# yardenas/ethz-safe-learning

Hardware: AMD Instinct MI355X
Metric: planning steps/sec (CEM-MPC, N=2000 K=5 H=30) (higher is better)
Workload: dtype f32

## Files before the change

### ethz_safe_learning_amd/_capi.py

```python
from __future__ import annotations

import ctypes as C
import os

CEM_ABI_VERSION = 4
CEM_MAX_ACT = 32
CEM_MAX_COST_KINDS = 4
CEM_COMM_ID_BYTES = 128
CEM_MAX_BATCH = 256
CEM_TRAIN_MAX_BATCH = 4096
CEM_INIT_COLD, CEM_INIT_EXPLICIT, CEM_INIT_SHIFT = 0, 1, 2
CEM_VARIANT_CEM, CEM_VARIANT_SAFE, CEM_VARIANT_COST = 0, 1, 2
CEM_PARTICLES_MEAN, CEM_PARTICLES_LOWER_TAIL = 0, 1
CEM_CONSTRAINT_BETA, CEM_CONSTRAINT_BUDGET = 0, 1
CEM_REFIT_UNIFORM, CEM_REFIT_SOFTMAX = 0, 1
CEM_NOISE_WHITE, CEM_NOISE_MIXED = 0, 1
CEM_FORWARD_SPLIT, CEM_FORWARD_ALL = 0, 1
CEM_TASK_SAFETY_GYM, CEM_TASK_QUADRATIC = 0, 1

_HERE = os.path.dirname(os.path.abspath(__file__))
LIB_PATH = os.environ.get('CEM_MPC_LIB') or os.path.join(_HERE, 'lib', 'libcem_mpc_gfx950.so')

EXPORTED_SYMBOLS = [
    'cem_abi_version', 'cem_status_string', 'cem_last_hip_error', 'cem_weight_blob_floats',
    'cem_packed_weight_floats', 'cem_workspace_bytes', 'cem_pack_weights_host', 'cem_plan_tiles_host', 'cem_plan_segments_host', 'cem_rollout_residency',
    'cem_planner_create', 'cem_planner_destroy', 'cem_planner_layout', 'cem_planner_set_weights', 'cem_planner_set_weights_dev',
    'cem_planner_set_normaliser', 'cem_planner_plan', 'cem_plan_begin', 'cem_plan_rollout', 'cem_plan_select',
    'cem_plan_end', 'cem_comm_unique_id', 'cem_planner_comm_init', 'cem_planner_comm_destroy', 'cem_planner_comm_ranks', 'cem_plan_exchange', 'cem_planner_graph_status', 'cem_planner_graph_nodes', 'cem_planner_launches_per_iteration', 'cem_planner_rollout_path', 'cem_planner_rollout_form', 'cem_unfold_sequences', 'cem_compute_objective', 'cem_scorer_reward', 'cem_scorer_cost', 'cem_fill_noise', 'cem_philox_words', 'cem_planner_set_timing', 'cem_planner_last_timing', 'cem_planner_last_timing_detail', 'cem_planner_select_mode', 'cem_planner_inject_fault',
    'cem_batch_workspace_bytes', 'cem_batch_planner_create', 'cem_planner_plan_batch', 'cem_planner_batch_capacity',
    'cem_planner_set_warm_start', 'cem_planner_set_initial_distribution', 'cem_planner_set_init_mode', 'cem_planner_reset_carry',
    'cem_planner_get_carry', 'cem_planner_set_carry_slots', 'cem_planner_set_particle_objective', 'cem_planner_get_particle_objective',
    'cem_planner_set_constraint', 'cem_planner_get_constraint', 'cem_planner_set_cost_budget', 'cem_planner_constraint_costs',
    'cem_planner_set_refit', 'cem_planner_get_refit', 'cem_planner_refit_stats',
    'cem_planner_set_action_noise', 'cem_planner_get_action_noise', 'cem_planner_action_noise_dev',
    'cem_planner_set_elite_carry', 'cem_planner_get_elite_carry', 'cem_planner_elite_store',
    'cem_planner_set_population_schedule', 'cem_planner_get_population_schedule', 'cem_planner_iteration_plan',
    'cem_planner_set_mean_candidate', 'cem_planner_get_mean_candidate',
    'cem_planner_set_plan_readout', 'cem_planner_get_plan_readout', 'cem_planner_plan_readout',
    'cem_planner_set_task', 'cem_planner_task_trajectories', 'cem_task_score',
    'cem_trainer_workspace_bytes', 'cem_trainer_blob_floats', 'cem_trainer_create', 'cem_trainer_destroy', 'cem_trainer_set_state',
    'cem_trainer_get_state', 'cem_trainer_weights_dev', 'cem_trainer_step', 'cem_trainer_steps', 'cem_trainer_eval', 'cem_trainer_forward',
]

# ... 109 lines not shown
    lib.cem_planner_comm_init.argtypes = [vp, vp, C.c_int32, C.c_int32]
    lib.cem_planner_comm_destroy.argtypes = [vp]
    lib.cem_plan_exchange.argtypes = [vp]
    lib.cem_planner_graph_status.argtypes = [vp, i32p]
    lib.cem_planner_graph_nodes.argtypes = [vp, i32p]
    lib.cem_planner_comm_ranks.argtypes = [vp, i32p]
    lib.cem_planner_launches_per_iteration.argtypes = [vp, i32p]
    lib.cem_planner_rollout_path.argtypes = [vp, i32p]
    lib.cem_planner_rollout_form.argtypes = [vp, C.c_int32, i32p]
    lib.cem_compute_objective.argtypes = [vp, vp, C.c_int32, C.c_int32, vp]
    lib.cem_scorer_reward.argtypes = [vp, vp, vp, C.c_int32, vp, vp]
    lib.cem_scorer_cost.argtypes = [vp, vp, C.c_int32, vp]
    lib.cem_fill_noise.argtypes = [vp, C.c_uint64, C.c_uint64, vp, vp, vp]
    lib.cem_philox_words.argtypes = [vp, C.c_uint64, C.c_uint64] + [C.c_uint32] * 6 + [vp]
    lib.cem_planner_select_mode.argtypes = [vp, i32p]
    lib.cem_planner_inject_fault.argtypes = [vp, C.c_int32]
    lib.cem_planner_set_timing.argtypes = [vp, C.c_int32]
    lib.cem_planner_last_timing.argtypes = [vp, fp, i32p, fp]
    lib.cem_planner_last_timing_detail.argtypes = [vp, fp, fp]
    lib.cem_batch_workspace_bytes.restype = C.c_size_t
    lib.cem_batch_workspace_bytes.argtypes = [cfgp, C.c_int32]
    lib.cem_batch_planner_create.argtypes = [cfgp, C.c_int32, vp, C.c_size_t, vp, C.POINTER(vp)]
    lib.cem_planner_plan_batch.argtypes = [vp, C.c_int32, vp, C.c_uint64, vp, vp, vp, vp, vp, vp, vp]
    lib.cem_planner_batch_capacity.argtypes = [vp, i32p]
    lib.cem_planner_set_warm_start.argtypes = [vp, C.POINTER(CemWarmStart)]
    lib.cem_planner_set_initial_distribution.argtypes = [vp, C.c_int32, vp, vp]
    lib.cem_planner_set_init_mode.argtypes = [vp, C.c_int32, C.c_int32]
    lib.cem_planner_reset_carry.argtypes = [vp, C.c_int32]
    lib.cem_planner_get_carry.argtypes = [vp, C.c_int32, vp, vp, i32p]
    lib.cem_planner_set_carry_slots.argtypes = [vp, C.c_int32, vp]
# ... 54 lines not shown
```

### ethz_safe_learning_amd/csrc/cem_capi.hip

```cpp
#include "cem_device.h"
#include "cem_rollout_lean.h"
#include "cem_score.h"
#include "cem_refit_weighted.h"
#include "cem_noise_mix.h"
#include "cem_elite_carry.h"
#include "cem_plan_readout.h"
#include "cem_task_score.h"
#include "cem_population.h"
#include "cem_train.h"
#include "cem_train_tile.h"
#include "cem_forward.h"
#include "cem_rollout_split.h"
#include "cem_rollout_bf16.h"
#include "cem_rollout_wide.h"
#include "cem_pack.h"
#include "../../include/cem_mpc.h"
#include "cem_plan_options.h"

#include <dlfcn.h>
#include <link.h>

#include <algorithm>
#include <atomic>
#include <chrono>
// ... 602 lines not shown
struct cem_planner {
    cem_config_t cfg;
    Dims d;
    Layout lay;
    char *ws;
    hipStream_t stream;
    bool own_stream;
    int rc;
    int n_tiles;
    int n_seg, seg_len, n_pinned;
    bool have_weights;
    bool in_plan;
    bool sample_in_rollout;
    bool lean_rollout;
    bool lean_branchy;
    const float *eps_act, *eps_model;
    CtrlBlock *h_ctrl;
    float *h_result;
    WarmCtl *h_warm; const WarmCtl *d_h_warm;
    uint32_t plan_seq;
    const CtrlBlock *d_h_ctrl; float *d_h_result;
    bool timing; std::vector<hipEvent_t> ev; float roll_ms, sel_ms, red_ms, samp_ms; int roll_n;
    std::vector<std::pair<int, int>> ev_kind;
    hipGraph_t graph; hipGraphExec_t gexec; bool graph_ready;
    ScorerDev sc;
    ScorerDev sc_roll;
    float alpha, beta;
    void *comm;
    int plans_since_comm;
    bool graph_failed;
    size_t sel_dyn_limit;
    int fused_resident;
    bool sel_zeroed;
    bool fuse_banned;
    bool inject_capture_fail;
    uint32_t inject_next;
    char *scratch; size_t scratch_bytes;
    std::vector<float> h_etab;
    PackDesc *pack_desc; uint32_t n_pack_desc;
    int batch;
    int n_states;
    cem_warm_start_t warm;
    std::vector<int32_t> slot_mode;
    std::vector<uint8_t> carry_valid, have_expl;
    std::vector<int32_t> carry_at;
    std::vector<int32_t> slot_of;
// ... 51 lines not shown
    return straight ? 2 : 1;
}
size_t task_tab_floats() { return (size_t)CEM_TASK_TABLES * CEM_U; }
float *task_traj(const cem_planner *h) { return h->task_dev + task_tab_floats(); }
int32_t *elite_counts(const cem_planner *h) { return reinterpret_cast<int32_t *>(h->elite_dev); }
size_t elite_count_floats(const cem_planner *h) { return ((size_t)warm_slots(h) + 63) & ~(size_t)63; }
float *elite_store(const cem_planner *h) { return h->elite_dev + elite_count_floats(h); }

int select_mode_for(const cem_planner *h, int N, bool *cache = nullptr)
{
    const Dims &d = h->d;
    const bool can_fuse = (N + CEM_MS_KEYS - 1) / CEM_MS_KEYS <= h->fused_resident && !h->fuse_banned;
    return resolve_select_mode(h->cfg.select_mode, N, d.k, (long long)d.H * d.A, h->sel_dyn_limit, can_fuse, cache);
}
int select_mode_now(const cem_planner *h, bool *cache = nullptr) { return select_mode_for(h, h->d.N, cache); }

void drop_graph(cem_planner *h)
{
    if (h->gexec) { hipGraphExecDestroy(h->gexec); h->gexec = nullptr; }
    if (h->graph) { hipGraphDestroy(h->graph); h->graph = nullptr; }
    h->graph_ready = false;
}

struct LaunchRecipe {
    bool sampler_launch;
    bool inject_elites, inject_mean;
    int lean_form;
    bool fold_reduce;
    int select_mode; bool select_cache;
    bool one_workgroup_only;
    bool weighted, keep_elites, track;
    bool task;
};
LaunchRecipe recipe_of(const cem_planner *h, int it, bool own_noise)
{
    const IterView v = iter_view(h, it); const PlanOptions &o = h->opt;
    LaunchRecipe r{};
    r.inject_elites = o.elite.n_keep != 0;
    r.inject_mean = o.mean_cand && it == h->d.I - 1;
    r.task = o.task != 0;
    const bool rewritten = r.inject_elites || r.inject_mean || r.task;
    r.sampler_launch = !v.sample_in_rollout || rewritten;
    r.lean_form = v.lean_rollout && !rewritten && !own_noise && o.noise_kind != CEM_NOISE_MIXED ? lean_form(h, it) : 0;
    r.select_mode = select_mode_for(h, v.d->N, &r.select_cache);
    r.fold_reduce = h->d.W == 1 && !h->comm && h->cfg.variant == CEM_VARIANT_CEM && !o.tail_m && r.select_mode == 1 && r.select_cache;
    r.weighted = o.refit_kind == CEM_REFIT_SOFTMAX; r.keep_elites = o.elite.n_keep != 0; r.track = o.readout != 0;
    r.one_workgroup_only = r.weighted || r.keep_elites || r.track || !h->pop.empty();
    return r;
}

int launches_of(const cem_planner *h, int it)
{
    const LaunchRecipe r = recipe_of(h, it, false);
    return 1 + r.sampler_launch + r.inject_elites + r.inject_mean + !r.fold_reduce + (r.select_mode == 2 ? 8 : r.select_mode == 3 ? 2 : 1) +
           r.weighted + r.keep_elites + r.track + r.task;
}

PlanOptions options_of(const cem_planner *h) { PlanOptions o = h->opt; o.comm = h->comm != nullptr; return o; }

// ... 177 lines not shown
    cem_planner *h = new (std::nothrow) cem_planner();
    if (!h) return CEM_ERR_INVALID_ARG;
    h->cfg = *cfg; h->d = make_dims(cfg);
    h->batch = mb; h->n_states = warm_slots(h);
    const size_t nb = (size_t)warm_slots(h);
    h->lay = make_layout(cfg, h->d, max_tiles_of(h->d), mb);
    if (workspace_bytes < h->lay.total || ((uintptr_t)workspace & 255)) { delete h; return CEM_ERR_WORKSPACE; }
    h->ws = (char *)workspace; h->stream = (hipStream_t)hip_stream; h->own_stream = false;
    if (!h->stream) {
        if (hipStreamCreateWithFlags(&h->stream, hipStreamNonBlocking) != hipSuccess) { g_last_hip = (int)hipGetLastError(); delete h; return CEM_ERR_HIP; }
        h->own_stream = true;
    }
    { const Plan pl = make_plan(cfg, h->d, mb); h->rc = pl.rc; h->n_seg = pl.n_seg; h->seg_len = pl.seg_len; h->n_pinned = pl.n_pinned;
      place_sampler(h, h->d, pl, &h->sample_in_rollout, &h->lean_rollout); }
    { const char *e = std::getenv("CEM_FORCE_ROLLOUT"); h->lean_branchy = e && std::strcmp(e, "lean_branchy") == 0; }
    h->have_weights = false; h->in_plan = false; h->eps_act = h->eps_model = nullptr;
    h->timing = false; h->roll_ms = h->sel_ms = h->red_ms = h->samp_ms = 0.f; h->roll_n = 0;
    h->graph = nullptr; h->gexec = nullptr; h->graph_ready = false;
    h->budget_dev = nullptr; h->cstat_obj = nullptr; h->cstat_obj_n = 0; h->last_cstat = nullptr; h->last_cstat_n = h->last_cstat_problems = 0;
    h->refit_beta = 0.f; h->refit_dev = nullptr; h->refit_ran = false;
    h->noise_dev = nullptr; h->noise_eps = nullptr; h->noise_floats = 0;
    h->elite_dev = nullptr; h->elite_cap = 0; h->elite_clear = false;
    h->readout_dev = nullptr;
    h->task_dev = nullptr; h->task = TaskScoreParams{};
    h->pop_dev = nullptr; h->pop_seg_flags = nullptr; h->pop_seg_state = nullptr; h->pop_n_ready = 0;
    h->h_budget.assign(nb, std::numeric_limits<float>::infinity());
    h->comm = nullptr; h->plans_since_comm = 0; h->graph_failed = false;
    h->h_ctrl = nullptr; h->h_result = nullptr; h->h_warm = nullptr; h->d_h_warm = nullptr; h->pack_desc = nullptr; h->n_pack_desc = 0;
    h->warm = cem_warm_start_t{}; h->warm.shift = 1; h->warm_staged = 0; h->warm_save_skipped = false;
    h->slot_mode.assign(nb, CEM_INIT_COLD); h->carry_valid.assign(nb, 0); h->have_expl.assign(nb, 0); h->carry_at.assign(nb, -1);
// ... 71 lines not shown
        !upload(h->lay.tiles, tiles.data(), tiles.size() * sizeof(Tile6)) || !upload(h->lay.omask, om.data(), om.size() * 4) ||
        !upload(h->lay.kind_sel, ks.data(), ks.size() * 4) || !upload(h->lay.nmin, mn.data(), CEM_U * 4) ||
        !upload(h->lay.ndelta, dl.data(), CEM_U * 4) || !upload(h->lay.etab, h->h_etab.data(), h->h_etab.size() * 4) ||
        hipMemsetAsync(h->ws + h->lay.act_pad, 0, nb * d.N * d.H * d.act_nq * 16, h->stream) != hipSuccess ||
        hipStreamSynchronize(h->stream) != hipSuccess)
        return fail(CEM_ERR_HIP);

    h->sel_dyn_limit = 48 * 1024;
    if (hipFuncSetAttribute(reinterpret_cast<const void *>(&cem_select_kernel<true, false>), hipFuncAttributeMaxDynamicSharedMemorySize,
                            140 * 1024) == hipSuccess &&
        hipFuncSetAttribute(reinterpret_cast<const void *>(&cem_select_kernel<true, true>), hipFuncAttributeMaxDynamicSharedMemorySize,
                            140 * 1024) == hipSuccess &&
        hipFuncSetAttribute(reinterpret_cast<const void *>(&cem_select_kernel<false, false>), hipFuncAttributeMaxDynamicSharedMemorySize,
                            140 * 1024) == hipSuccess) h->sel_dyn_limit = 140 * 1024;
    else (void)hipGetLastError();
    {
        int per_cu = 0;
        if (hipOccupancyMaxActiveBlocksPerMultiprocessor(&per_cu, cem_msel_fused_kernel, 1024, 0) != hipSuccess || per_cu < 1) { (void)hipGetLastError(); per_cu = 0; }
        h->fused_resident = per_cu * real_cus();
    }
    if (mb && select_mode_now(h) != 1) { release_handle(h); return CEM_ERR_UNSUPPORTED; }
    *out = h;
    return CEM_OK;
}

extern "C" {

int cem_planner_create(const cem_config_t *cfg, void *workspace, size_t workspace_bytes, void *hip_stream, cem_planner_t **out)
{
    return planner_create(cfg, 0, workspace, workspace_bytes, hip_stream, out);
// ... 421 lines not shown
            hipLaunchKernelGGL(cem_msel_hist_kernel<2>, dim3(m.G), dim3(1024), 0, h->stream, m);
            hipLaunchKernelGGL(cem_msel_count_kernel, dim3(m.G), dim3(1024), 0, h->stream, m);
            hipLaunchKernelGGL(cem_msel_compact_kernel, dim3(m.G), dim3(1024), 0, h->stream, m);
            hipLaunchKernelGGL(cem_msel_moments_kernel<0>, dim3(m.G2), dim3(256), 0, h->stream, m);
            hipLaunchKernelGGL(cem_msel_moments_kernel<1>, dim3(m.G2), dim3(256), 0, h->stream, m);
            hipLaunchKernelGGL(cem_msel_final_kernel, dim3(1), dim3(256), 0, h->stream, m);
        }
    } else {
        if (fold_final && !h->batch && !weighted) {
            p.is_last = it == d.I - 1;
            p.result = h->d_h_result; p.result_dev = (uint32_t *)(ws + l.result); p.eps_out = have_eps_out ? (const float *)(ws + l.eps_out) : nullptr; p.noise_stddev = h->cfg.noise_stddev;
            if (folded) *folded = true;
        }
        if (cache) lds += (size_t)CEM_SEL_KWORDS(d.N) * 4;
        const dim3 grid(warm_slots(h));
        if (cache && h->cfg.variant != CEM_VARIANT_CEM) hipLaunchKernelGGL((cem_select_kernel<true, true>), grid, dim3(1024), lds, h->stream, p);
        else if (cache) hipLaunchKernelGGL((cem_select_kernel<true, false>), grid, dim3(1024), lds, h->stream, p);
        else hipLaunchKernelGGL((cem_select_kernel<false, false>), grid, dim3(1024), lds, h->stream, p);
        if (weighted) {
            HIPCHK(hipGetLastError());
            RefitWeightedParams rw{}; rw.scores = p.scores; rw.actions = p.actions; rw.musig = (float *)(ws + l.musig); rw.ctrl = p.ctrl; rw.elite_idx = p.elite_idx;
            rw.stat = h->refit_dev + (size_t)warm_slots(h) * 2 * p.HA;
            rw.N = d.N; rw.k = d.k; rw.HA = p.HA; rw.I = d.I; rw.beta = h->refit_beta;
            rw.smoothing = p.smoothing; rw.one_minus_smoothing = p.one_minus_smoothing; rw.threshold = h->cfg.stddev_threshold;
            HIPCHK(launch_refit_weighted(rw, warm_slots(h), h->stream));
            h->refit_ran = true;
        }
        if (rc.keep_elites) {
            HIPCHK(hipGetLastError());
            const EliteCarryParams ep = fill_elite(h, it);
            HIPCHK(launch_elite_keep(ep, warm_slots(h), h->stream));
// ... 1066 lines not shown
    WordsParams wp{}; wp.out = words_out_dev; wp.ctrl = (const CtrlBlock *)(h->ws + h->lay.ctrl);
    wp.stream = stream; wp.it = iteration; wp.t = t; wp.sub = sub; wp.idx0 = idx0; wp.n = n;
    hipLaunchKernelGGL(cem_philox_words_kernel, dim3((n + 255) / 256), dim3(256), 0, h->stream, wp);
    HIPCHK(hipGetLastError());
    HIPCHK(hipStreamSynchronize(h->stream));
    return CEM_OK;
}

int cem_planner_select_mode(const cem_planner_t *h, int32_t *mode_out)
{
    if (!h || !mode_out) return CEM_ERR_INVALID_ARG;
    *mode_out = select_mode_now(h);
    return CEM_OK;
}

int cem_planner_inject_fault(cem_planner_t *h, int32_t kind)
{
    if (!h || (kind != 1 && kind != 2)) return CEM_ERR_INVALID_ARG;
    if (h->in_plan) return CEM_ERR_STATE;
    if (kind == 2) { h->inject_capture_fail = true; return CEM_OK; }
    h->inject_next = 1u;
    return CEM_OK;
}

int cem_planner_set_timing(cem_planner_t *h, int32_t enable)
{
    if (!h) return CEM_ERR_INVALID_ARG;
    h->timing = enable != 0;
    return CEM_OK;
}
// ... 308 lines not shown
```

### ethz_safe_learning_amd/csrc/cem_device.h

```cpp
#pragma once
#include <hip/hip_runtime.h>
#include <stdint.h>

typedef float f4 __attribute__((ext_vector_type(4)));

#define CEM_U 128
#define CEM_ET_NMIN 0
#define CEM_ET_RDELTA 1
#define CEM_ET_BMU 2
#define CEM_ET_BVAR 3
#define CEM_ET_OBS 4
#define CEM_ET_ACT 5
#define CEM_ET_SEL0 6
#define CEM_ET_SEL1 7
#define CEM_ET_ROWS 8
#define CEM_NG 8
#define CEM_NKIND 5
#define CEM_PART_FLOATS (CEM_NKIND * 4 * 64)
#define CEM_TAB_LDS_BYTES (CEM_ET_ROWS * CEM_U * 4)
#define CEM_ROLLOUT_LDS_BYTES(RC_) ((size_t)2 * (RC_) * CEM_NG * 1024 + CEM_PART_FLOATS * 4 + CEM_TAB_LDS_BYTES)

struct TileDesc {
    int32_t row_base;
    int32_t cnt;
// ... 918 lines not shown
        return;
    }
    const float d = cem_goal_dist16(o, p.sc, j), dn = cem_goal_dist16(p.next_obs + (size_t)row * p.O, p.sc, j);
    const bool ga = d <= p.sc.goal_thresh;
    const float r = cem_reward_of(d, dn, ga, p.sc);
    if (j == 0) { p.out[row] = r; if (p.flag) p.flag[row] = ga ? 1 : 0; }
}

__device__ __forceinline__ float cem_out_noise(const CtrlBlock *ctrl, const float *eps_out, const int a)
{
    if (eps_out) return eps_out[a];
    const f4 e = cem_normal4((uint32_t)(a >> 2), 0u, 0u, 0u, CEM_STREAM_OUT, cem_key(ctrl));
    return e[a & 3];
}


#define CEM_RESULT_WORDS 38
#define CEM_RESULT_MAGIC 0x5EC0DE5Au
__host__ __device__ inline uint32_t cem_result_checksum(const volatile uint32_t *w, const uint32_t seq)
{
    uint32_t x = CEM_RESULT_MAGIC ^ seq;
    for (int i = 0; i < 36; ++i) x = (x ^ w[i]) * 0x01000193u;
    return x ^ (x >> 15);
}
__device__ __forceinline__ void cem_emit_result(float *result, uint32_t *result_dev, const uint32_t *res_l , const uint32_t seq, const int lane)
{
    const uint32_t x = cem_result_checksum(res_l, seq);
    if (lane < CEM_RESULT_WORDS) {
        const uint32_t w = lane < 36 ? res_l[lane] : (lane == 36 ? seq : x);
        if (result_dev) result_dev[lane] = w;
// ... 28 lines not shown
    for (int round = 0; round < 4 && rem; ++round) {
        const int leader = __builtin_ctzll(rem);
        const uint32_t d = (uint32_t)__builtin_amdgcn_readlane((int)digit, leader);
        const uint64_t same = __builtin_amdgcn_ballot_w64(match && digit == d);
        if (lane == leader) atomicAdd(&hist[d], (uint32_t)__builtin_popcountll(same));
        rem &= ~same;
        if ((same >> lane) & 1ull) match = false;
    }
    if (match) atomicAdd(&hist[digit], 1u);
}

__device__ __forceinline__ float cem_key2f(const uint32_t key)
{
    return __uint_as_float((key & 0x80000000u) ? (key ^ 0x80000000u) : ~key);
}

__device__ __forceinline__ void cem_block_excl_scan2(const uint32_t a, const uint32_t b, uint32_t (*wsum)[16], uint32_t &pa, uint32_t &pb)
{
    const int lane = threadIdx.x & 63, wv = threadIdx.x >> 6;
    uint32_t ia = a, ib = b;
#pragma unroll
    for (int d = 1; d < 64; d <<= 1) {
        const uint32_t oa = __shfl_up(ia, d), ob = __shfl_up(ib, d);
        if (lane >= d) { ia += oa; ib += ob; }
    }
    if (lane == 63) { wsum[0][wv] = ia; wsum[1][wv] = ib; }
    __syncthreads();
    uint32_t ba = 0, bb = 0;
    for (int i = 0; i < wv; ++i) { ba += wsum[0][i]; bb += wsum[1][i]; }
    pa = ba + ia - a; pb = bb + ib - b;
// ... 974 lines not shown
```

### ethz_safe_learning_amd/planner.py

```python
from __future__ import annotations

import ctypes as C
import math
from dataclasses import dataclass, field
from typing import List, NamedTuple, Optional, Sequence, Tuple

import numpy as np

from . import _capi


@dataclass
class ScorerConfig:
    goal_slice: Tuple[int, int]
    observe_goal_lidar: bool = True
    lidar_max_dist: float = 4.0
    goal_size: float = 0.3
    reward_distance: float = 1.0
    reward_goal: float = 1.0
    reward_clip: float = 10.0
    constrain_indicator: bool = True
    cost_kinds: List[Tuple[int, int, float]] = field(default_factory=list)


# ... 649 lines not shown
            raise ValueError('actions must be [rows / particles, H, act_dim]')
        ret = t.empty((B,), dtype=t.float32, device=self.device)
        costs = t.empty((H, B), dtype=t.uint8, device=self.device) if c.variant != 'cem' else None
        self._wait_inputs()
        _capi.check(self.lib.cem_task_score(self.h, _ptr(traj), _ptr(act), B, H, _ptr(ret), _ptr(costs)), 'cem_task_score')
        return ret, costs

    def plan_exchange(self):
        _capi.check(self.lib.cem_plan_exchange(self.h), 'cem_plan_exchange')

    def select_mode(self):
        m = C.c_int32()
        _capi.check(self.lib.cem_planner_select_mode(self.h, C.byref(m)), 'cem_planner_select_mode')
        return m.value

    def inject_fault(self, kind=1):
        _capi.check(self.lib.cem_planner_inject_fault(self.h, kind), 'cem_planner_inject_fault')

    INIT_MODES = {'cold': _capi.CEM_INIT_COLD, 'explicit': _capi.CEM_INIT_EXPLICIT, 'shift': _capi.CEM_INIT_SHIFT}

    def n_slots(self):
        return self.max_batch

    def set_warm_start(self, shift=1, tail='box', sigma='reset', floor_frac=0.0):
        tails, rules = {'box': 0, 'repeat': 1}, {'reset': 0, 'keep': 1}
        if tail not in tails or sigma not in rules:
            raise ValueError("tail is 'box' or 'repeat', sigma is 'reset' or 'keep'")
        ws = _capi.CemWarmStart(shift=int(shift), tail=tails[tail], sigma_rule=rules[sigma])
        ws.sigma_floor[:self.cfg.act_dim] = warm_sigma_floor(self.cfg, floor_frac).tolist()
        _capi.check(self.lib.cem_planner_set_warm_start(self.h, C.byref(ws)), 'cem_planner_set_warm_start')
# ... 556 lines not shown
```

### include/cem_mpc.h

```cpp
#ifndef CEM_MPC_H
#define CEM_MPC_H

#include <stddef.h>
#include <stdint.h>

#ifdef __cplusplus
extern "C" {
#endif

#define CEM_ABI_VERSION 4
#define CEM_MAX_ACT 32
#define CEM_MAX_COST_KINDS 4
#define CEM_MAX_BATCH 256

enum cem_status {
    CEM_OK = 0,
    CEM_ERR_INVALID_ARG = 1,
    CEM_ERR_UNSUPPORTED = 2,
    CEM_ERR_SPLIT = 3,
    CEM_ERR_WORKSPACE = 4,
    CEM_ERR_HIP = 5,
    CEM_ERR_NO_WEIGHTS = 6,
    CEM_ERR_STATE = 7,
    CEM_ERR_COMM = 8,
// ... 99 lines not shown
                     float *action_out, float *best_score_out, int32_t *iters_out);

int cem_plan_begin(cem_planner_t *h, const float *state, uint64_t seed, uint64_t call,
                   const float *eps_act_dev, const float *eps_model_dev);
int cem_plan_rollout(cem_planner_t *h, int32_t it);
int cem_plan_select(cem_planner_t *h, int32_t it);
int cem_plan_end(cem_planner_t *h, const float *eps_out_host, float *action_out, float *best_score_out, int32_t *iters_out);

#define CEM_COMM_ID_BYTES 128
int cem_comm_unique_id(void *id_out );
int cem_planner_comm_init(cem_planner_t *h, const void *id , int32_t n_ranks, int32_t rank);
int cem_planner_comm_destroy(cem_planner_t *h);
int cem_planner_comm_ranks(const cem_planner_t *h, int32_t *n_ranks_out);
int cem_plan_exchange(cem_planner_t *h);
int cem_planner_select_mode(const cem_planner_t *h, int32_t *mode_out);
int cem_planner_inject_fault(cem_planner_t *h, int32_t kind);
int cem_planner_graph_status(const cem_planner_t *h, int32_t *status_out);
int cem_planner_graph_nodes(const cem_planner_t *h, int32_t *nodes_out);
int cem_planner_launches_per_iteration(const cem_planner_t *h, int32_t *launches_out);
int cem_planner_rollout_path(const cem_planner_t *h, int32_t *path_out);
int cem_planner_rollout_form(const cem_planner_t *h, int32_t it, int32_t *form_out);

int cem_unfold_sequences(cem_planner_t *h, const float *s0_dev, const float *actions_dev, int32_t n_rows, int32_t horizon,
                         const float *eps_model_dev, uint64_t seed, uint64_t call,
                         float *traj_out_dev, float *mu_out_dev, float *sd_out_dev);

int cem_compute_objective(cem_planner_t *h, const float *traj_dev, int32_t n_rows, int32_t horizon, float *scores_out_dev);

int cem_scorer_reward(cem_planner_t *h, const float *obs_dev, const float *next_obs_dev, int32_t n, float *reward_out_dev,
                      uint8_t *goal_achieved_out_dev);
// ... 130 lines not shown
```

Before: 552.1.

## Add register-resident radix-select elite kernel for plain CEM selection

```diff
diff --git a/ethz_safe_learning_amd/_capi.py b/ethz_safe_learning_amd/_capi.py
--- a/ethz_safe_learning_amd/_capi.py
+++ b/ethz_safe_learning_amd/_capi.py
@@ -27,6 +27,7 @@
     'cem_planner_create', 'cem_planner_destroy', 'cem_planner_layout', 'cem_planner_set_weights', 'cem_planner_set_weights_dev',
     'cem_planner_set_normaliser', 'cem_planner_plan', 'cem_plan_begin', 'cem_plan_rollout', 'cem_plan_select',
     'cem_plan_end', 'cem_comm_unique_id', 'cem_planner_comm_init', 'cem_planner_comm_destroy', 'cem_planner_comm_ranks', 'cem_plan_exchange', 'cem_planner_graph_status', 'cem_planner_graph_nodes', 'cem_planner_launches_per_iteration', 'cem_planner_rollout_path', 'cem_planner_rollout_form', 'cem_unfold_sequences', 'cem_compute_objective', 'cem_scorer_reward', 'cem_scorer_cost', 'cem_fill_noise', 'cem_philox_words', 'cem_planner_set_timing', 'cem_planner_last_timing', 'cem_planner_last_timing_detail', 'cem_planner_select_mode', 'cem_planner_inject_fault',
+    'cem_planner_select_form', 'cem_select_form_for',
     'cem_batch_workspace_bytes', 'cem_batch_planner_create', 'cem_planner_plan_batch', 'cem_planner_batch_capacity',
     'cem_planner_set_warm_start', 'cem_planner_set_initial_distribution', 'cem_planner_set_init_mode', 'cem_planner_reset_carry',
     'cem_planner_get_carry', 'cem_planner_set_carry_slots', 'cem_planner_set_particle_objective', 'cem_planner_get_particle_objective',
@@ -166,6 +167,8 @@
     lib.cem_fill_noise.argtypes = [vp, C.c_uint64, C.c_uint64, vp, vp, vp]
     lib.cem_philox_words.argtypes = [vp, C.c_uint64, C.c_uint64] + [C.c_uint32] * 6 + [vp]
     lib.cem_planner_select_mode.argtypes = [vp, i32p]
+    lib.cem_planner_select_form.argtypes = [vp, C.c_int32, i32p]
+    lib.cem_select_form_for.argtypes = [C.c_int32, C.c_int64, C.c_int64, C.c_int64, C.c_int32, i32p]
     lib.cem_planner_inject_fault.argtypes = [vp, C.c_int32]
     lib.cem_planner_set_timing.argtypes = [vp, C.c_int32]
     lib.cem_planner_last_timing.argtypes = [vp, fp, i32p, fp]
diff --git a/ethz_safe_learning_amd/csrc/cem_capi.hip b/ethz_safe_learning_amd/csrc/cem_capi.hip
--- a/ethz_safe_learning_amd/csrc/cem_capi.hip
+++ b/ethz_safe_learning_amd/csrc/cem_capi.hip
@@ -5,6 +5,7 @@
 #include "cem_noise_mix.h"
 #include "cem_elite_carry.h"
 #include "cem_plan_readout.h"
+#include "cem_select_ranked.h"
 #include "cem_task_score.h"
 #include "cem_population.h"
 #include "cem_train.h"
@@ -640,6 +641,7 @@
     bool sample_in_rollout;
     bool lean_rollout;
     bool lean_branchy;
+    bool select_bucket;
     const float *eps_act, *eps_model;
     CtrlBlock *h_ctrl;
     float *h_result;
@@ -656,6 +658,7 @@
     int plans_since_comm;
     bool graph_failed;
     size_t sel_dyn_limit;
+    bool ranked_ready;
     int fused_resident;
     bool sel_zeroed;
     bool fuse_banned;
@@ -737,6 +740,11 @@
     return resolve_select_mode(h->cfg.select_mode, N, d.k, (long long)d.H * d.A, h->sel_dyn_limit, can_fuse, cache);
 }
 int select_mode_now(const cem_planner *h, bool *cache = nullptr) { return select_mode_for(h, h->d.N, cache); }
+int select_form_of(const cem_planner *h, int mode, bool cache, int N)
+{
+    if (!h->ranked_ready || h->select_bucket) return 0;
+    return select_ranked_form(mode, cache, N, h->cfg.variant == CEM_VARIANT_CEM);
+}
 
 void drop_graph(cem_planner *h)
 {
@@ -751,6 +759,7 @@
     int lean_form;
     bool fold_reduce;
     int select_mode; bool select_cache;
+    int select_form;
     bool one_workgroup_only;
     bool weighted, keep_elites, track;
     bool task;
@@ -766,6 +775,7 @@
     r.sampler_launch = !v.sample_in_rollout || rewritten;
     r.lean_form = v.lean_rollout && !rewritten && !own_noise && o.noise_kind != CEM_NOISE_MIXED ? lean_form(h, it) : 0;
     r.select_mode = select_mode_for(h, v.d->N, &r.select_cache);
+    r.select_form = select_form_of(h, r.select_mode, r.select_cache, v.d->N);
     r.fold_reduce = h->d.W == 1 && !h->comm && h->cfg.variant == CEM_VARIANT_CEM && !o.tail_m && r.select_mode == 1 && r.select_cache;
     r.weighted = o.refit_kind == CEM_REFIT_SOFTMAX; r.keep_elites = o.elite.n_keep != 0; r.track = o.readout != 0;
     r.one_workgroup_only = r.weighted || r.keep_elites || r.track || !h->pop.empty();
@@ -973,6 +983,7 @@
     { const Plan pl = make_plan(cfg, h->d, mb); h->rc = pl.rc; h->n_seg = pl.n_seg; h->seg_len = pl.seg_len; h->n_pinned = pl.n_pinned;
       place_sampler(h, h->d, pl, &h->sample_in_rollout, &h->lean_rollout); }
     { const char *e = std::getenv("CEM_FORCE_ROLLOUT"); h->lean_branchy = e && std::strcmp(e, "lean_branchy") == 0; }
+    { const char *e = std::getenv("CEM_FORCE_SELECT"); h->select_bucket = e && std::strcmp(e, "bucket") == 0; }
     h->have_weights = false; h->in_plan = false; h->eps_act = h->eps_model = nullptr;
     h->timing = false; h->roll_ms = h->sel_ms = h->red_ms = h->samp_ms = 0.f; h->roll_n = 0;
     h->graph = nullptr; h->gexec = nullptr; h->graph_ready = false;
@@ -1074,6 +1085,8 @@
         hipFuncSetAttribute(reinterpret_cast<const void *>(&cem_select_kernel<false, false>), hipFuncAttributeMaxDynamicSharedMemorySize,
                             140 * 1024) == hipSuccess) h->sel_dyn_limit = 140 * 1024;
     else (void)hipGetLastError();
+    h->ranked_ready = launch_select_ranked && prepare_select_ranked && prepare_select_ranked(h->sel_dyn_limit) == hipSuccess;
+    if (!h->ranked_ready) (void)hipGetLastError();
     {
         int per_cu = 0;
         if (hipOccupancyMaxActiveBlocksPerMultiprocessor(&per_cu, cem_msel_fused_kernel, 1024, 0) != hipSuccess || per_cu < 1) { (void)hipGetLastError(); per_cu = 0; }
@@ -1525,7 +1538,8 @@
         }
         if (cache) lds += (size_t)CEM_SEL_KWORDS(d.N) * 4;
         const dim3 grid(warm_slots(h));
-        if (cache && h->cfg.variant != CEM_VARIANT_CEM) hipLaunchKernelGGL((cem_select_kernel<true, true>), grid, dim3(1024), lds, h->stream, p);
+        if (rc.select_form == 1) HIPCHK(launch_select_ranked(p, warm_slots(h), lds, h->stream));
+        else if (cache && h->cfg.variant != CEM_VARIANT_CEM) hipLaunchKernelGGL((cem_select_kernel<true, true>), grid, dim3(1024), lds, h->stream, p);
         else if (cache) hipLaunchKernelGGL((cem_select_kernel<true, false>), grid, dim3(1024), lds, h->stream, p);
         else hipLaunchKernelGGL((cem_select_kernel<false, false>), grid, dim3(1024), lds, h->stream, p);
         if (weighted) {
@@ -2622,6 +2636,22 @@
     return CEM_OK;
 }
 
+int cem_planner_select_form(const cem_planner_t *h, int32_t it, int32_t *form_out)
+{
+    if (!h || !form_out || it < 0 || it >= h->d.I) return CEM_ERR_INVALID_ARG;
+    *form_out = recipe_of(h, it, false).select_form;
+    return CEM_OK;
+}
+
+int cem_select_form_for(int32_t select_mode, int64_t n_samples, int64_t n_elite, int64_t horizon_x_act_dim, int32_t variant, int32_t *form_out)
+{
+    if (!form_out || select_mode < 0 || select_mode > 3 || n_samples < 1 || n_elite < 1 || n_elite > n_samples || horizon_x_act_dim < 1) return CEM_ERR_INVALID_ARG;
+    bool cache = false;
+    const int mode = resolve_select_mode(select_mode, n_samples, n_elite, horizon_x_act_dim, 140 * 1024, true, &cache);
+    *form_out = select_ranked_form(mode, cache, n_samples, variant == CEM_VARIANT_CEM);
+    return CEM_OK;
+}
+
 int cem_planner_inject_fault(cem_planner_t *h, int32_t kind)
 {
     if (!h || (kind != 1 && kind != 2)) return CEM_ERR_INVALID_ARG;
diff --git a/ethz_safe_learning_amd/csrc/cem_device.h b/ethz_safe_learning_amd/csrc/cem_device.h
--- a/ethz_safe_learning_amd/csrc/cem_device.h
+++ b/ethz_safe_learning_amd/csrc/cem_device.h
@@ -956,6 +956,7 @@
     return e[a & 3];
 }
 
+#endif
 
 #define CEM_RESULT_WORDS 38
 #define CEM_RESULT_MAGIC 0x5EC0DE5Au
@@ -1014,6 +1015,8 @@
 {
     return __uint_as_float((key & 0x80000000u) ? (key ^ 0x80000000u) : ~key);
 }
+
+#ifndef CEM_DEVICE_PRIMITIVES_ONLY
 
 __device__ __forceinline__ void cem_block_excl_scan2(const uint32_t a, const uint32_t b, uint32_t (*wsum)[16], uint32_t &pa, uint32_t &pb)
 {
diff --git a/ethz_safe_learning_amd/csrc/cem_select_ranked.h b/ethz_safe_learning_amd/csrc/cem_select_ranked.h
--- /dev/null
+++ b/ethz_safe_learning_amd/csrc/cem_select_ranked.h
@@ -0,0 +1,12 @@
+#pragma once
+#include "cem_device.h"
+
+#define CEM_SELECT_RANKED_MAX_N 4096
+
+inline int select_ranked_form(const int mode, const bool cache, const long long N, const bool plain)
+{
+    return mode == 1 && cache && N <= CEM_SELECT_RANKED_MAX_N && plain ? 1 : 0;
+}
+
+__attribute__((weak)) hipError_t prepare_select_ranked(size_t bytes);
+__attribute__((weak)) hipError_t launch_select_ranked(const SelectParams &p, int n_problems, size_t lds_bytes, hipStream_t st);
diff --git a/ethz_safe_learning_amd/csrc/cem_select_ranked.hip b/ethz_safe_learning_amd/csrc/cem_select_ranked.hip
--- /dev/null
+++ b/ethz_safe_learning_amd/csrc/cem_select_ranked.hip
@@ -0,0 +1,378 @@
+#define CEM_DEVICE_PRIMITIVES_ONLY
+#include "cem_select_ranked.h"
+
+#define CEM_SR_LIST_MAX 256u
+
+#define CEM_SR_DPP(ID, V, CTRL, ROWS) ((uint32_t)__builtin_amdgcn_update_dpp((int)(ID), (int)(V), (CTRL), (ROWS), 0xf, false))
+#define CEM_SR_WAVE_STEPS(OP, ID, V) do { \
+        V = OP(V, CEM_SR_DPP(ID, V, 0x111, 0xf)); V = OP(V, CEM_SR_DPP(ID, V, 0x112, 0xf)); \
+        V = OP(V, CEM_SR_DPP(ID, V, 0x114, 0xf)); V = OP(V, CEM_SR_DPP(ID, V, 0x118, 0xf)); \
+        V = OP(V, CEM_SR_DPP(ID, V, 0x142, 0xa)); V = OP(V, CEM_SR_DPP(ID, V, 0x143, 0xc)); } while (0)
+__device__ __forceinline__ uint32_t cem_sr_add(const uint32_t a, const uint32_t b) { return a + b; }
+__device__ __forceinline__ uint32_t cem_sr_min(const uint32_t a, const uint32_t b) { return a < b ? a : b; }
+__device__ __forceinline__ uint32_t cem_sr_max(const uint32_t a, const uint32_t b) { return a > b ? a : b; }
+__device__ __forceinline__ uint32_t cem_sr_wave_scan(uint32_t v) { CEM_SR_WAVE_STEPS(cem_sr_add, 0u, v); return v; }
+__device__ __forceinline__ uint32_t cem_sr_wave_min(uint32_t v) { CEM_SR_WAVE_STEPS(cem_sr_min, 0xFFFFFFFFu, v); return (uint32_t)__builtin_amdgcn_readlane((int)v, 63); }
+__device__ __forceinline__ uint32_t cem_sr_wave_max(uint32_t v) { CEM_SR_WAVE_STEPS(cem_sr_max, 0u, v); return (uint32_t)__builtin_amdgcn_readlane((int)v, 63); }
+
+__device__ __forceinline__ uint32_t cem_sr_below(const uint64_t b) { return __builtin_amdgcn_mbcnt_hi((uint32_t)(b >> 32), __builtin_amdgcn_mbcnt_lo((uint32_t)b, 0u)); }
+
+__device__ __forceinline__ void cem_sr_find(const uint32_t cnt, const uint32_t need, int &b, uint32_t &need_in, uint32_t &m)
+{
+    const uint32_t inc = cem_sr_wave_scan(cnt);
+    const uint32_t gt = (uint32_t)__builtin_amdgcn_readlane((int)inc, 63) - inc;
+    const uint64_t who = __builtin_amdgcn_ballot_w64(gt < need && need <= gt + cnt);
+    b = who ? __builtin_ctzll(who) : 0;
+    need_in = need - (uint32_t)__builtin_amdgcn_readlane((int)gt, b);
+    m = (uint32_t)__builtin_amdgcn_readlane((int)cnt, b);
+}
+
+__device__ __forceinline__ void cem_sr_offsets(const uint32_t *tot, const int lane, const int wv, uint32_t off[4])
+{
+    const uint32_t v = tot[lane], ex = cem_sr_wave_scan(v) - v;
+    const int w = __builtin_amdgcn_readfirstlane(wv);
+#pragma unroll
+    for (int j = 0; j < 4; ++j) off[j] = (uint32_t)__builtin_amdgcn_readlane((int)ex, 16 * j + w);
+}
+
+__global__ __launch_bounds__(1024) void cem_select_ranked_kernel(const SelectParams p)
+{
+    extern __shared__ __attribute__((aligned(16))) char sel_smem[];
+    __shared__ __attribute__((aligned(16))) float red[4096];
+    __shared__ __attribute__((aligned(16))) uint32_t wmm[2][16];
+    __shared__ __attribute__((aligned(16))) uint32_t wtot[64];
+    __shared__ __attribute__((aligned(16))) uint32_t etot[64];
+    __shared__ __attribute__((aligned(16))) uint32_t coarse[64];
+    __shared__ uint32_t sh_cnt;
+    __shared__ int sh_best;
+    const int prob = (int)blockIdx.x;
+    CtrlBlock *const ctrl = p.ctrl + prob;
+    const int done = p.check_done ? __hip_atomic_load(&ctrl->done, __ATOMIC_RELAXED, __HIP_MEMORY_SCOPE_WORKGROUP) : 0;
+    const float *const scores_b = p.scores + (size_t)prob * p.N;
+    const float *const actions_b = p.actions + (size_t)prob * p.N * p.HA;
+    float *const musig_b = p.musig + (size_t)prob * 2 * p.HA;
+    int32_t *const elite_b = p.elite_idx + (size_t)prob * p.k;
+    const float *const ret_b = p.ret ? p.ret + (size_t)prob * p.P * p.N : p.ret;
+    float *const scores_wb = p.scores_w ? p.scores_w + (size_t)prob * p.N : p.scores_w;
+
+    const int tid = threadIdx.x, lane = tid & 63, wv = tid >> 6;
+    const int N = p.N, k = p.k, HA = p.HA;
+    CEM_SEL_STAMP(0);
+    int32_t *elite = reinterpret_cast<int32_t *>(sel_smem);
+    float *colmean = reinterpret_cast<float *>(sel_smem + (size_t)((k + 3) & ~3) * 4);
+    float *newsig = colmean + HA;
+    uint32_t *h2k = reinterpret_cast<uint32_t *>(red);
+    uint32_t *lkey = h2k + 2048, *lidx = lkey + 1024;
+
+    float old_mu = 0.f, old_sg = 0.f;
+    if (tid < HA) { old_mu = musig_b[tid]; old_sg = musig_b[HA + tid]; }
+
+    float v[4] = {0.f, 0.f, 0.f, 0.f};
+    if (ret_b) {
+        float acc[4] = {0.f, 0.f, 0.f, 0.f};
+        for (int q0 = 0; q0 < p.P; q0 += 8) {
+            float r[8][4];
+#pragma unroll
+            for (int j = 0; j < 4; ++j)
+                if (j * 1024 < N) {
+                    const int i = j * 1024 + tid, ic = i < N ? i : N - 1;
+#pragma unroll
+                    for (int u = 0; u < 8; ++u) r[u][j] = ret_b[(size_t)(q0 + u < p.P ? q0 + u : p.P - 1) * N + ic];
+                }
+#pragma unroll
+            for (int u = 0; u < 8; ++u)
+                if (q0 + u < p.P) {
+#pragma unroll
+                    for (int j = 0; j < 4; ++j) if (j * 1024 < N) acc[j] = acc[j] + r[u][j];
+                }
+        }
+#pragma unroll
+        for (int j = 0; j < 4; ++j) v[j] = acc[j] / (float)p.P;
+    } else {
+#pragma unroll
+        for (int j = 0; j < 4; ++j) { const int i = j * 1024 + tid; if (i < N) v[j] = scores_b[i]; }
+    }
+    uint32_t key[4];
+    uint32_t play = 0u;
+    uint32_t kmin = 0xFFFFFFFFu, kmax = 0u;
+#pragma unroll
+    for (int j = 0; j < 4; ++j) {
+        const bool in = j * 1024 + tid < N;
+        key[j] = in ? cem_f2key(v[j]) : 0u;
+        if (in) { play |= 1u << j; kmin = key[j] < kmin ? key[j] : kmin; kmax = key[j] > kmax ? key[j] : kmax; }
+    }
+    kmin = cem_sr_wave_min(kmin); kmax = cem_sr_wave_max(kmax);
+    if (lane == 0) { wmm[0][wv] = kmin; wmm[1][wv] = kmax; }
+    h2k[tid] = 0u; h2k[tid + 1024] = 0u;
+    if (tid < 64) coarse[tid] = 0u;
+    if (tid == 0) { sh_cnt = 0u; sh_best = 0x7fffffff; }
+    for (int e = tid; e < k; e += 1024) elite[e] = 0;
+    __syncthreads();
+    if (__builtin_amdgcn_readfirstlane(done)) return;
+    kmin = cem_sr_wave_min(wmm[0][lane & 15]); kmax = cem_sr_wave_max(wmm[1][lane & 15]);
+    if (scores_wb) {
+#pragma unroll
+        for (int j = 0; j < 4; ++j) if ((play >> j) & 1u) scores_wb[j * 1024 + tid] = v[j];
+    }
+    {
+        int mine = 0x7fffffff;
+#pragma unroll
+        for (int j = 3; j >= 0; --j) if (((play >> j) & 1u) && key[j] == kmax) mine = j * 1024 + tid;
+        if (mine != 0x7fffffff) atomicMin(&sh_best, mine);
+    }
+    CEM_SEL_STAMP(1);
+
+    uint32_t base = kmin, need = (uint32_t)k;
+    int sh; { const uint32_t window = kmax - kmin; sh = window ? max(0, 21 - (int)__clz((int)window)) : 0; }
+    uint32_t take = 0u;
+    uint32_t need1 = 0u, m = 0u;
+#pragma unroll 1
+    for (int level = 0; level < 4; ++level) {
+        if (level) {
+            __syncthreads();
+            h2k[tid] = 0u; h2k[tid + 1024] = 0u;
+            if (tid < 64) coarse[tid] = 0u;
+            __syncthreads();
+        }
+#pragma unroll
+        for (int j = 0; j < 4; ++j)
+            if ((play >> j) & 1u) { const uint32_t b = (key[j] - base) >> sh; atomicAdd(&h2k[b], 1u); atomicAdd(&coarse[b >> 5], 1u); }
+        __syncthreads();
+        int grp, q;
+        uint32_t need_in, unused;
+        cem_sr_find(coarse[lane], need, grp, need_in, unused);
+        cem_sr_find(lane < 32 ? h2k[grp * 32 + lane] : 0u, need_in, q, need1, m);
+        const uint32_t bucket = (uint32_t)(grp * 32 + q);
+#pragma unroll
+        for (int j = 0; j < 4; ++j)
+            if ((play >> j) & 1u) {
+                const uint32_t b = (key[j] - base) >> sh;
+                if (b > bucket) take |= 1u << j;
+                if (b != bucket) play &= ~(1u << j);
+            }
+        if (sh == 0 || m <= CEM_SR_LIST_MAX || need1 >= m) break;
+        base += bucket << sh; need = need1;
+        sh = sh > 11 ? sh - 11 : 0;
+    }
+    if (need1 >= m) take |= play;
+    else if (sh == 0) {
+        uint64_t eb[4];
+#pragma unroll
+        for (int j = 0; j < 4; ++j) {
+            eb[j] = __builtin_amdgcn_ballot_w64(((play >> j) & 1u) != 0u);
+            if (lane == 0) etot[16 * j + wv] = (uint32_t)__builtin_popcountll(eb[j]);
+        }
+        __syncthreads();
+        uint32_t off[4];
+        cem_sr_offsets(etot, lane, wv, off);
+#pragma unroll
+        for (int j = 0; j < 4; ++j)
+            if (((play >> j) & 1u) && off[j] + cem_sr_below(eb[j]) < need1) take |= 1u << j;
+    } else {
+#pragma unroll
+        for (int j = 0; j < 4; ++j)
+            if ((play >> j) & 1u) {
+                const uint32_t pos = atomicAdd(&sh_cnt, 1u);
+                if (pos < 1024u) { lkey[pos] = key[j]; lidx[pos] = (uint32_t)(j * 1024 + tid); }
+            }
+        __syncthreads();
+        if (play) {
+            uint32_t before[4] = {0u, 0u, 0u, 0u};
+            for (uint32_t l = 0; l < m; ++l) {
+                const uint32_t kl = lkey[l], il = lidx[l];
+#pragma unroll
+                for (int j = 0; j < 4; ++j) before[j] += (kl > key[j]) || (kl == key[j] && il < (uint32_t)(j * 1024 + tid));
+            }
+#pragma unroll
+            for (int j = 0; j < 4; ++j) if (((play >> j) & 1u) && before[j] < need1) take |= 1u << j;
+        }
+    }
+    CEM_SEL_STAMP(2);
+
+    {
+        uint64_t tb[4];
+#pragma unroll
+        for (int j = 0; j < 4; ++j) {
+            tb[j] = __builtin_amdgcn_ballot_w64(((take >> j) & 1u) != 0u);
+            if (lane == 0) wtot[16 * j + wv] = (uint32_t)__builtin_popcountll(tb[j]);
+        }
+        __syncthreads();
+        uint32_t off[4];
+        cem_sr_offsets(wtot, lane, wv, off);
+#pragma unroll
+        for (int j = 0; j < 4; ++j)
+            if ((take >> j) & 1u) {
+                const uint32_t pos = off[j] + cem_sr_below(tb[j]);
+                if (pos < (uint32_t)k) { elite[pos] = j * 1024 + tid; elite_b[pos] = j * 1024 + tid; }
+            }
+    }
+    __syncthreads();
+
+    CEM_SEL_STAMP(3);
+
+    CEM_SEL_STAMP(4);
+    const float fk = (float)k;
+    const float sm = p.smoothing, osm = p.one_minus_smoothing;
+    int tpc1 = 1; { const int nc = HA < 1024 ? HA : 1024; while (tpc1 * 2 * nc <= 1024) tpc1 *= 2; }
+    if ((HA & 3) == 0 && HA <= 4096 && k > 16 * tpc1) {
+        const int ncol4 = HA >> 2;
+        int tpc = 1; while (tpc * 2 * ncol4 <= 1024) tpc *= 2;
+        const int part = tid / ncol4, c4 = tid % ncol4;
+        const bool act = part < tpc;
+        f4 *red4 = reinterpret_cast<f4 *>(red);
+        const f4 *act4 = reinterpret_cast<const f4 *>(actions_b);
+        const f4 zero4 = (f4){0.f, 0.f, 0.f, 0.f};
+        f4 av[8];
+#pragma unroll
+        for (int j = 0; j < 8; ++j) {
+            const int e = part + j * tpc;
+            av[j] = (act && e < k) ? act4[(size_t)elite[e] * ncol4 + c4] : zero4;
+        }
+        f4 mean4 = zero4;
+        for (int phase = 0; phase < 2; ++phase) {
+            f4 acc = zero4;
+            if (act) {
+#pragma unroll
+                for (int j = 0; j < 8; ++j)
+                    if (part + j * tpc < k) { const f4 a = av[j]; acc = phase ? acc + (a - mean4) * (a - mean4) : acc + a; }
+                for (int e0 = part + 8 * tpc; e0 < k; e0 += 8 * tpc) {
+                    f4 b[8];
+#pragma unroll
+                    for (int j = 0; j < 8; ++j) { const int e = e0 + j * tpc; b[j] = e < k ? act4[(size_t)elite[e] * ncol4 + c4] : zero4; }
+#pragma unroll
+                    for (int j = 0; j < 8; ++j)
+                        if (e0 + j * tpc < k) { const f4 a = b[j]; acc = phase ? acc + (a - mean4) * (a - mean4) : acc + a; }
+                }
+            }
+            __syncthreads();
+            red4[tid] = acc;
+            __syncthreads();
+            if (part == 0) {
+                f4 tot = zero4;
+                for (int pp = 0; pp < tpc; ++pp) tot = tot + red4[pp * ncol4 + c4];
+                if (!phase) {
+#pragma unroll
+                    for (int r = 0; r < 4; ++r) colmean[4 * c4 + r] = tot[r] / fk;
+                } else {
+#pragma unroll
+                    for (int r = 0; r < 4; ++r) {
+                        const float sd = sqrtf(tot[r] / fk);
+                        const int ci = 4 * c4 + r;
+                        const float nsg = sm * musig_b[HA + ci] + osm * sd;
+                        musig_b[ci] = sm * musig_b[ci] + osm * colmean[ci];
+                        musig_b[HA + ci] = nsg;
+                        newsig[ci] = nsg;
+                    }
+                }
+            }
+            __syncthreads();
+            if (!phase && act) {
+#pragma unroll
+                for (int r = 0; r < 4; ++r) mean4[r] = colmean[4 * c4 + r];
+            }
+        }
+    } else {
+        for (int cb = 0; cb < HA; cb += 1024) {
+            const int ncol = (HA - cb < 1024) ? HA - cb : 1024;
+            int tpc = 1; while (tpc * 2 * ncol <= 1024) tpc *= 2;
+            const int part = tid / ncol, col = tid % ncol;
+            const bool act = part < tpc;
+            float av[16];
+#pragma unroll
+            for (int j = 0; j < 16; ++j) {
+                const int e = part + j * tpc;
+                av[j] = (act && e < k) ? actions_b[(size_t)elite[e] * HA + cb + col] : 0.f;
+            }
+            for (int phase = 0; phase < 2; ++phase) {
+                float acc = 0.f;
+                const float mc = phase ? colmean[cb + col] : 0.f;
+                if (act) {
+#pragma unroll
+                    for (int j = 0; j < 16; ++j) {
+                        const int e = part + j * tpc;
+                        if (e < k) { const float a = av[j]; acc = phase ? acc + (a - mc) * (a - mc) : acc + a; }
+                    }
+                    for (int e0 = part + 16 * tpc; e0 < k; e0 += 8 * tpc) {
+                        float b[8];
+#pragma unroll
+                        for (int j = 0; j < 8; ++j) { const int e = e0 + j * tpc; b[j] = e < k ? actions_b[(size_t)elite[e] * HA + cb + col] : 0.f; }
+#pragma unroll
+                        for (int j = 0; j < 8; ++j)
+                            if (e0 + j * tpc < k) { const float a = b[j]; acc = phase ? acc + (a - mc) * (a - mc) : acc + a; }
+                    }
+                }
+                __syncthreads();
+                red[tid] = acc;
+                __syncthreads();
+                if (part == 0) {
+                    float tot = 0.f;
+                    for (int pp = 0; pp < tpc; ++pp) tot = tot + red[pp * ncol + col];
+                    if (!phase) colmean[cb + col] = tot / fk;
+                    else {
+                        const float sd = sqrtf(tot / fk);
+                        const int ci = cb + col;
+                        const float omu = cb == 0 ? old_mu : musig_b[ci], osg = cb == 0 ? old_sg : musig_b[HA + ci];
+                        const float nsg = sm * osg + osm * sd;
+                        musig_b[ci] = sm * omu + osm * colmean[ci];
+                        musig_b[HA + ci] = nsg;
+                        newsig[ci] = nsg;
+                    }
+                }
+                __syncthreads();
+            }
+        }
+    }
+    CEM_SEL_STAMP(5);
+    uint32_t *res_l = reinterpret_cast<uint32_t *>(red);
+    if (p.result && tid < 37) res_l[tid] = 0u;
+    if (p.result) __syncthreads();
+    if (tid == 0) {
+        float ssum = 0.f;
+        for (int i = 0; i < HA; ++i) ssum = ssum + newsig[i];
+        const float mean_sigma = ssum / (float)HA;
+        const int iters = ctrl->iters + 1;
+        const bool stop = mean_sigma <= p.threshold;
+        ctrl->iters = iters;
+        if (stop) ctrl->done = 1;
+        if (p.result) {
+            res_l[33] = (uint32_t)iters; res_l[34] = stop ? 1u : (uint32_t)ctrl->done; res_l[35] = (uint32_t)ctrl->fault;
+            res_l[36] = (stop || p.is_last != 0) ? 1u : 0u;
+        }
+        CEM_SEL_STAMP(6);
+    }
+    if (tid == 64) {
+        const float bs = cem_key2f(kmax);
+        const int idx = (uint32_t)sh_best < (uint32_t)N ? sh_best : 0;
+        const bool better = bs > ctrl->best_score;
+        for (int a0 = 0; a0 < p.A; a0 += 4) {
+            f4 e = (f4){0.f, 0.f, 0.f, 0.f};
+            if (p.result && !p.eps_out) e = cem_normal4((uint32_t)(a0 >> 2), 0u, 0u, 0u, CEM_STREAM_OUT, cem_key(ctrl));
+#pragma unroll
+            for (int r = 0; r < 4; ++r) {
+                const int a = a0 + r;
+                if (a < p.A) {
+                    const float b = better ? actions_b[(size_t)idx * HA + a] : ctrl->best[a];
+                    if (better) ctrl->best[a] = b;
+                    if (p.result) res_l[a] = __float_as_uint(b + (p.eps_out ? p.eps_out[a] : e[r]) * p.noise_stddev);
+                }
+            }
+        }
+        if (better) ctrl->best_score = bs;
+        if (p.result) res_l[32] = __float_as_uint(better ? bs : ctrl->best_score);
+    }
+    if (p.result) {
+        __syncthreads();
+        if (tid < 64 && res_l[36]) cem_emit_result(p.result, p.result_dev, res_l, ctrl->seq, tid);
+    }
+}
+
+hipError_t prepare_select_ranked(size_t bytes)
+{
+    return hipFuncSetAttribute(reinterpret_cast<const void *>(&cem_select_ranked_kernel), hipFuncAttributeMaxDynamicSharedMemorySize, (int)bytes);
+}
+
+hipError_t launch_select_ranked(const SelectParams &p, int n_problems, size_t lds_bytes, hipStream_t st)
+{
+    hipLaunchKernelGGL(cem_select_ranked_kernel, dim3(n_problems), dim3(1024), lds_bytes, st, p);
+    return hipGetLastError();
+}
diff --git a/ethz_safe_learning_amd/planner.py b/ethz_safe_learning_amd/planner.py
--- a/ethz_safe_learning_amd/planner.py
+++ b/ethz_safe_learning_amd/planner.py
@@ -687,6 +687,11 @@
         _capi.check(self.lib.cem_planner_select_mode(self.h, C.byref(m)), 'cem_planner_select_mode')
         return m.value
 
+    def select_form(self, it=0):
+        n = C.c_int32()
+        _capi.check(self.lib.cem_planner_select_form(self.h, int(it), C.byref(n)), 'cem_planner_select_form')
+        return n.value
+
     def inject_fault(self, kind=1):
         _capi.check(self.lib.cem_planner_inject_fault(self.h, kind), 'cem_planner_inject_fault')
 
diff --git a/include/cem_mpc.h b/include/cem_mpc.h
--- a/include/cem_mpc.h
+++ b/include/cem_mpc.h
@@ -137,6 +137,8 @@
 int cem_planner_comm_ranks(const cem_planner_t *h, int32_t *n_ranks_out);
 int cem_plan_exchange(cem_planner_t *h);
 int cem_planner_select_mode(const cem_planner_t *h, int32_t *mode_out);
+int cem_planner_select_form(const cem_planner_t *h, int32_t it, int32_t *form_out);
+int cem_select_form_for(int32_t select_mode, int64_t n_samples, int64_t n_elite, int64_t horizon_x_act_dim, int32_t variant, int32_t *form_out);
 int cem_planner_inject_fault(cem_planner_t *h, int32_t kind);
 int cem_planner_graph_status(const cem_planner_t *h, int32_t *status_out);
 int cem_planner_graph_nodes(const cem_planner_t *h, int32_t *nodes_out);
```

New measurement: 558.8 (median of 6 runs). 1.2% higher.
